# MicahZoltu/lodestar

Measured on AMD Instinct MI355X. Metric: verified signature sets/sec (mainnet attestation mix), higher is better.
Workload: dtype u32 (381-bit Montgomery; device products on 14x28-bit limbs); 1 GPU; c3: gossip attestation flood, 6 slot(s) per batch, 7 batches in flight per GPU; slots_per_batch=6, sets_per_gpu=116736, jobs_per_gpu=104448, pubkeys_per_gpu=1683456, parallelism=dp1 (sets sharded), exchange=False, inflight=7, world_size_seen=1, pubkeys=indices into the GPU-resident table, signing_roots_per_gpu=6918

## Files before the change

lodestar_amd/csrc/lb_curve.h:

```cpp
#pragma once
#include "lb_field.h"

template <class F>
struct jac {
  F x, y, z;
};
template <class F>
struct aff {
  F x, y;
};

typedef jac<fp> g1j;
typedef jac<fp2> g2j;
typedef aff<fp> g1a;
typedef aff<fp2> g2a;

template <class T, class S>
LB_HD aff<T> aff_as(const aff<S>& a) {
  return aff<T>{T{a.x}, T{a.y}};
}
template <class T, class S>
LB_HD jac<T> jac_as(const jac<S>& a) {
  return jac<T>{T{a.x}, T{a.y}, T{a.z}};
}
// ... 214 lines not shown
  }
  return acc;
}

template <class F>
LB_NI jac<F> jac_mul_u64_jac(jac<F> p, uint64_t k) {
  jac<F> acc = jac_infinity<F>();
  for (int i = 63; i >= 0; i--) {
    acc = jac_dbl_i(acc);
    if ((k >> i) & 1ull) acc = jac_add_i(acc, p);
  }
  return acc;
}

template <class F>
LB_NI jac<F> jac_mul_u256(aff<F> p, const uint32_t* k) {
  jac<F> acc = jac_infinity<F>();
  for (int i = 255; i >= 0; i--) {
    acc = jac_dbl_i(acc);
    if ((k[i >> 5] >> (i & 31)) & 1u) acc = jac_add_aff_i(acc, p);
  }
  return acc;
}

template <class F, bool kInl = false>
LB_HD jac<F> jac_mul_xabs_i(const jac<F>& p) {
  jac<F> acc = p;
  for (int i = 62; i >= 0; i--) {
    acc = jac_dbl_i(acc);
    if ((LB_X_ABS >> i) & 1ull) acc = jac_add_i<F, kInl>(acc, p);
  }
  return acc;
}
template <class F>
LB_NI jac<F> jac_mul_xabs(jac<F> p) {
  return jac_mul_xabs_i(p);
}

LB_HD g2j g2_psi(const g2j& p) {
  g2j r;
  r.x = fp2_mul(fp2_conj(p.x), fp2_load(LB_PSI_CX));
  r.y = fp2_mul(fp2_conj(p.y), fp2_load(LB_PSI_CY));
  r.z = fp2_conj(p.z);
  return r;
}
LB_HD g2j g2_psi2(const g2j& p) {
  g2j r;
  r.x = fp2_mul_fp(p.x, fp_load(LB_PSI2_CX));
  r.y = fp2_mul_fp(p.y, fp_load(LB_PSI2_CY));
  r.z = p.z;
  return r;
}

LB_HD bool g2_in_subgroup(const g2j& p) {
  if (jac_is_inf(p)) return true;
  g2j xp = jac_neg(jac_mul_xabs(p));
  return jac_eq(g2_psi(p), xp);
}

template <bool kInl>
LB_HD fp lean_mul(const fp& a, const fp& b) {
#if defined(__HIP_DEVICE_COMPILE__)
  if constexpr (kInl) {
    __builtin_amdgcn_sched_barrier(0);
    fp r = fp_mul28(a, b);
    __builtin_amdgcn_sched_barrier(0);
    return r;
  }
#endif
  return fp_mul(a, b);
}
template <bool kInl>
LB_HD fp lean_sqr(const fp& a) {
#if defined(__HIP_DEVICE_COMPILE__)
  if constexpr (kInl) {
    __builtin_amdgcn_sched_barrier(0);
    fp r = fp_sqr28(a);
    __builtin_amdgcn_sched_barrier(0);
    return r;
  }
#endif
  return fp_sqr(a);
}
template <bool kInl>
LB_HD fp2 lean2_mul(const fp2& a, const fp2& b) {
  fp t0 = lean_mul<kInl>(a.c0, b.c0);
  fp t1 = lean_mul<kInl>(a.c1, b.c1);
  fp t2 = lean_mul<kInl>(fp_add(a.c0, a.c1), fp_add(b.c0, b.c1));
  return fp2{fp_sub(t0, t1), fp_sub(fp_sub(t2, t0), t1)};
}
template <bool kInl>
LB_HD fp2 lean2_sqr(const fp2& a) {
  fp t0 = lean_mul<kInl>(fp_add(a.c0, a.c1), fp_sub(a.c0, a.c1));
  fp t1 = lean_mul<kInl>(a.c0, a.c1);
  return fp2{t0, fp_dbl(t1)};
}
template <bool kInl>
LB_HD void g2_dbl_lean(g2j& p) {
  p.z = fp2_dbl(lean2_mul<kInl>(p.y, p.z));
  fp2 B = lean2_sqr<kInl>(p.y);
  fp2 C = lean2_sqr<kInl>(B);
  fp2 A = lean2_sqr<kInl>(p.x);
  fp2 D = lean2_sqr<kInl>(fp2_add(p.x, B));
  D = fp2_dbl(fp2_sub(fp2_sub(D, A), C));
  fp2 E = fp2_mul3(A);
  p.x = fp2_sub(lean2_sqr<kInl>(E), fp2_dbl(D));
  p.y = fp2_sub(lean2_mul<kInl>(E, fp2_sub(D, p.x)), fp2_mul8(C));
}
template <bool kInl>
LB_HD void g2_add_aff_lean(g2j& p, const g2a& q) {
  fp2 Z1Z1 = lean2_sqr<kInl>(p.z);
  fp2 H = fp2_sub(lean2_mul<kInl>(q.x, Z1Z1), p.x);
  fp2 rr = lean2_mul<kInl>(lean2_mul<kInl>(q.y, p.z), Z1Z1);
  rr = fp2_dbl(fp2_sub(rr, p.y));
  if (fp2_is_zero(H)) {
    if (fp2_is_zero(rr)) {
      g2_dbl_lean<kInl>(p);
    } else {
      p = jac_infinity<fp2>();
    }
    return;
  }
  fp2 HH = lean2_sqr<kInl>(H);
  p.z = fp2_sub(fp2_sub(lean2_sqr<kInl>(fp2_add(p.z, H)), Z1Z1), HH);
  fp2 I = fp2_mul4(HH);
  fp2 J = lean2_mul<kInl>(H, I);
  fp2 V = lean2_mul<kInl>(p.x, I);
  fp2 YJ = fp2_dbl(lean2_mul<kInl>(p.y, J));
  p.x = fp2_sub(fp2_sub(lean2_sqr<kInl>(rr), J), fp2_dbl(V));
  p.y = fp2_sub(lean2_mul<kInl>(rr, fp2_sub(V, p.x)), YJ);
}

template <bool kInl>
LB_HD void g2_add_lean(g2j& p, const g2j& q) {
  if (jac_is_inf(q)) return;
  if (jac_is_inf(p)) {
    p = q;
    return;
  }
  const fp2 Z1Z1 = lean2_sqr<kInl>(p.z), Z2Z2 = lean2_sqr<kInl>(q.z);
  const fp2 ZZ = fp2_sub(fp2_sub(lean2_sqr<kInl>(fp2_add(p.z, q.z)), Z1Z1), Z2Z2);
  const fp2 U1 = lean2_mul<kInl>(p.x, Z2Z2);
  const fp2 S1 = lean2_mul<kInl>(lean2_mul<kInl>(p.y, q.z), Z2Z2);
  const fp2 H = fp2_sub(lean2_mul<kInl>(q.x, Z1Z1), U1);
  const fp2 rr = fp2_dbl(fp2_sub(lean2_mul<kInl>(lean2_mul<kInl>(q.y, p.z), Z1Z1), S1));
  if (fp2_is_zero(H)) {
    if (fp2_is_zero(rr)) {
      p = q;
      g2_dbl_lean<kInl>(p);
    } else {
      p = jac_infinity<fp2>();
    }
    return;
  }
  p.z = lean2_mul<kInl>(ZZ, H);
  const fp2 I = lean2_sqr<kInl>(fp2_dbl(H));
  const fp2 J = lean2_mul<kInl>(H, I);
  const fp2 V = lean2_mul<kInl>(U1, I);
  p.x = fp2_sub(fp2_sub(lean2_sqr<kInl>(rr), J), fp2_dbl(V));
  p.y = fp2_sub(lean2_mul<kInl>(rr, fp2_sub(V, p.x)), fp2_dbl(lean2_mul<kInl>(S1, J)));
}

LB_HD bool g2_aff_in_subgroup_i(const g2a& a) {
  g2j acc = jac_from_aff(a);
#pragma clang loop unroll(disable)
  for (int i = 62; i >= 0; i--) {
    acc = jac_dbl_i(acc);
    if ((LB_X_ABS >> i) & 1ull) acc = jac_add_aff_i<fp2, true>(acc, a);
  }
  if (jac_is_inf(acc)) return false;
  fp2 z2 = fp2_sqr(acc.z);
  fp2 px = fp2_mul(fp2_conj(a.x), fp2_load(LB_PSI_CX));
  if (!fp2_eq(fp2_mul(px, z2), acc.x)) return false;
  fp2 py = fp2_mul(fp2_conj(a.y), fp2_load(LB_PSI_CY));
  return fp2_eq(fp2_mul(fp2_mul(py, z2), acc.z), fp2_neg(acc.y));
}

LB_NI g2j g2_clear_cofactor(g2j p) {
  g2j t1 = jac_neg(jac_mul_xabs(p));
  g2j t2 = g2_psi(p);
  g2j t3 = g2_psi2(jac_dbl(p));
  t3 = jac_add(t3, jac_neg(t2));
  t2 = jac_add(t1, t2);
  t2 = jac_neg(jac_mul_xabs(t2));
  t3 = jac_add(t3, t2);
  t3 = jac_add(t3, jac_neg(t1));
  return jac_add(t3, jac_neg(p));
}

LB_HD bool g1_aff_on_curve(const g1a& a) {
// ... 6 lines not shown
```

lodestar_amd/csrc/lb_field.h:

```cpp
#pragma once
#include "lb_common.h"
#include "lb_consts.h"

struct fp {
  uint32_t v[12];
};
struct fp2 {
  fp c0, c1;
};
struct fp6 {
  fp2 c0, c1, c2;
};
struct fp12 {
  fp6 c0, c1;
};

LB_HD fp fp_load(const uint32_t* c) {
  fp r;
  LB_UNROLL for (int i = 0; i < 12; i++) r.v[i] = c[i];
  return r;
}
LB_HD fp2 fp2_load(const uint32_t* c) {
  fp2 r;
  r.c0 = fp_load(c);
// ... 681 lines not shown
    }
    lb_sub_in(u, v);
    bool zero = true;
    LB_UNROLL for (int j = 0; j < 12; j++) zero &= u[j] == 0;
    if (zero) return false;
  }
}

LB_HD bool fp_plain_gt_half(const fp& plain) {
  uint32_t br = 0;
  LB_UNROLL for (int j = 0; j < 12; j++) {
    uint64_t d = (uint64_t)LB_HALF_P[j] - plain.v[j] - br;
    br = (uint32_t)(d >> 63);
  }
  return br != 0;
}

LB_HD bool fp_plain_from_be48(fp& out, const uint8_t* b, uint8_t first_byte_mask) {
  LB_UNROLL for (int i = 0; i < 12; i++) {
    int o = 44 - 4 * i;
    uint32_t b0 = b[o];
    if (i == 11) b0 &= first_byte_mask;
    out.v[i] = (b0 << 24) | ((uint32_t)b[o + 1] << 16) | ((uint32_t)b[o + 2] << 8) | b[o + 3];
  }
  const uint32_t Pl[12] = {LB_P0, LB_P1, LB_P2, LB_P3, LB_P4, LB_P5, LB_P6, LB_P7, LB_P8, LB_P9, LB_P10, LB_P11};
  uint32_t br = 0;
  LB_UNROLL for (int j = 0; j < 12; j++) {
    uint64_t d = (uint64_t)out.v[j] - Pl[j] - br;
    br = (uint32_t)(d >> 63);
  }
  return br != 0;
}

LB_HD uint32_t lb_bswap32(uint32_t x) { return (x >> 24) | ((x >> 8) & 0xff00u) | ((x << 8) & 0xff0000u) | (x << 24); }
LB_HD bool fp_plain_from_be48_w(fp& out, const uint32_t* w, uint8_t first_byte_mask) {
  LB_UNROLL for (int i = 0; i < 12; i++) out.v[i] = lb_bswap32(w[11 - i]);
  out.v[11] &= ((uint32_t)first_byte_mask << 24) | 0x00ffffffu;
  const uint32_t Pl[12] = {LB_P0, LB_P1, LB_P2, LB_P3, LB_P4, LB_P5, LB_P6, LB_P7, LB_P8, LB_P9, LB_P10, LB_P11};
  uint32_t br = 0;
  LB_UNROLL for (int j = 0; j < 12; j++) {
    uint64_t d = (uint64_t)out.v[j] - Pl[j] - br;
    br = (uint32_t)(d >> 63);
  }
  return br != 0;
}

LB_HD void fp_plain_to_be48(uint8_t* b, const fp& plain) {
  LB_UNROLL for (int i = 0; i < 12; i++) {
    int o = 44 - 4 * i;
    uint32_t w = plain.v[i];
    b[o] = (uint8_t)(w >> 24);
    b[o + 1] = (uint8_t)(w >> 16);
    b[o + 2] = (uint8_t)(w >> 8);
    b[o + 3] = (uint8_t)w;
  }
}

LB_HD fp2 fp2_zero() { return fp2{fp_zero(), fp_zero()}; }
LB_HD fp2 fp2_one() { return fp2{fp_one(), fp_zero()}; }
LB_HD bool fp2_is_zero(const fp2& a) { return fp_is_zero(a.c0) && fp_is_zero(a.c1); }
LB_HD bool fp2_eq(const fp2& a, const fp2& b) { return fp_eq(a.c0, b.c0) && fp_eq(a.c1, b.c1); }
LB_HD fp2 fp2_select(bool c, const fp2& a, const fp2& b) { return fp2{fp_select(c, a.c0, b.c0), fp_select(c, a.c1, b.c1)}; }
LB_HD fp2 fp2_add(const fp2& a, const fp2& b) { return fp2{fp_add(a.c0, b.c0), fp_add(a.c1, b.c1)}; }
LB_HD fp2 fp2_sub(const fp2& a, const fp2& b) { return fp2{fp_sub(a.c0, b.c0), fp_sub(a.c1, b.c1)}; }
LB_HD fp2 fp2_dbl(const fp2& a) { return fp2{fp_dbl(a.c0), fp_dbl(a.c1)}; }
LB_HD fp2 fp2_neg(const fp2& a) { return fp2{fp_neg(a.c0), fp_neg(a.c1)}; }
LB_HD fp2 fp2_conj(const fp2& a) { return fp2{a.c0, fp_neg(a.c1)}; }
LB_HD fp2 fp2_mul_fp(const fp2& a, const fp& s) { return fp2{fp_mul(a.c0, s), fp_mul(a.c1, s)}; }
LB_HD fp2 fp2_mul3(const fp2& a) { return fp2{fp_mul3(a.c0), fp_mul3(a.c1)}; }
LB_HD fp2 fp2_mul4(const fp2& a) { return fp2{fp_mul4(a.c0), fp_mul4(a.c1)}; }
LB_HD fp2 fp2_mul8(const fp2& a) { return fp2{fp_mul8(a.c0), fp_mul8(a.c1)}; }

LB_HD fp2 fp2_mul(const fp2& a, const fp2& b) {
  fp t0 = fp_mul(a.c0, b.c0);
  fp t1 = fp_mul(a.c1, b.c1);
  fp t2 = fp_mul(fp_add(a.c0, a.c1), fp_add(b.c0, b.c1));
  return fp2{fp_sub(t0, t1), fp_sub(fp_sub(t2, t0), t1)};
}
LB_HD fp2 fp2_sqr(const fp2& a) {
  fp t0 = fp_mul(fp_add(a.c0, a.c1), fp_sub(a.c0, a.c1));
  fp t1 = fp_mul(a.c0, a.c1);
  return fp2{t0, fp_dbl(t1)};
}
LB_HD fp2 fp2_mul_xi(const fp2& a) { return fp2{fp_sub(a.c0, a.c1), fp_add(a.c0, a.c1)}; }

LB_NI fp2 fp2_inv(fp2 a) {
  fp n = fp_add(fp_sqr(a.c0), fp_sqr(a.c1));
  fp ni = fp_inv(n);
  return fp2{fp_mul(a.c0, ni), fp_neg(fp_mul(a.c1, ni))};
}

LB_HD bool fp2_is_square(const fp2& a) { return fp_is_square(fp_add(fp_sqr(a.c0), fp_sqr(a.c1))); }

template <bool kInl = false>
LB_HD bool fp2_sqrt_i(fp2& out, const fp2& a) {
  fp norm = fp_add(fp_sqr(a.c0), fp_sqr(a.c1));
  fp alpha;
  if constexpr (kInl) alpha = fp_pow_const_i<true>(norm, LB_EXP_SQRT, 378);
  else alpha = fp_sqrt_cand(norm);
  fp inv2 = fp_load(LB_INV2);
  fp d1 = fp_mul(fp_add(a.c0, alpha), inv2);
  fp d2 = fp_mul(fp_sub(a.c0, alpha), inv2);
  fp delta = fp_select(fp_is_zero(d1), d2, d1);
  fp z;
  if constexpr (kInl) z = fp_pow_const_i<true>(delta, LB_EXP_ISQRT, 378);
  else z = fp_isqrt_cand(delta);
  fp s = fp_mul(delta, z);
  bool delta_qr = fp_eq(fp_sqr(s), delta);
  fp t = fp_mul(z, inv2);
  if (!delta_qr) t = fp_neg(t);
  fp q = fp_mul(a.c1, t);
  out.c0 = fp_select(delta_qr, s, q);
  out.c1 = fp_select(delta_qr, q, s);
  return fp2_eq(fp2_sqr(out), a);
}
LB_NI bool fp2_sqrt(fp2& out, fp2 a) { return fp2_sqrt_i(out, a); }
template <class Pow>
LB_HD bool fp2_sqrt_p(fp2& out, const fp2& a, Pow pow) {
  const fp norm = fp_add(fp_sqr(a.c0), fp_sqr(a.c1));
  const fp alpha = pow(norm, LB_EXP_SQRT, 378);
  const fp inv2 = fp_load(LB_INV2);
  const fp d1 = fp_mul(fp_add(a.c0, alpha), inv2);
  const fp d2 = fp_mul(fp_sub(a.c0, alpha), inv2);
  const fp delta = fp_select(fp_is_zero(d1), d2, d1);
  const fp z = pow(delta, LB_EXP_ISQRT, 378);
  const fp s = fp_mul(delta, z);
  const bool delta_qr = fp_eq(fp_sqr(s), delta);
  fp t = fp_mul(z, inv2);
  if (!delta_qr) t = fp_neg(t);
  const fp q = fp_mul(a.c1, t);
  out.c0 = fp_select(delta_qr, s, q);
  out.c1 = fp_select(delta_qr, q, s);
  return fp2_eq(fp2_sqr(out), a);
}

LB_HD uint32_t fp2_sgn0(const fp2& a) {
  fp p0 = fp_from_mont(a.c0), p1 = fp_from_mont(a.c1);
  uint32_t sign0 = p0.v[0] & 1u;
  uint32_t zero0 = fp_is_zero(p0) ? 1u : 0u;
  uint32_t sign1 = p1.v[0] & 1u;
  return sign0 | (zero0 & sign1);
}

LB_HD bool fp2_lex_larger(const fp2& a) {
  fp p0 = fp_from_mont(a.c0), p1 = fp_from_mont(a.c1);
  return fp_is_zero(p1) ? fp_plain_gt_half(p0) : fp_plain_gt_half(p1);
}

LB_HD fp6 fp6_zero() { return fp6{fp2_zero(), fp2_zero(), fp2_zero()}; }
LB_HD fp6 fp6_one() { return fp6{fp2_one(), fp2_zero(), fp2_zero()}; }
LB_HD fp6 fp6_add(const fp6& a, const fp6& b) { return fp6{fp2_add(a.c0, b.c0), fp2_add(a.c1, b.c1), fp2_add(a.c2, b.c2)}; }
LB_HD fp6 fp6_sub(const fp6& a, const fp6& b) { return fp6{fp2_sub(a.c0, b.c0), fp2_sub(a.c1, b.c1), fp2_sub(a.c2, b.c2)}; }
LB_HD fp6 fp6_neg(const fp6& a) { return fp6{fp2_neg(a.c0), fp2_neg(a.c1), fp2_neg(a.c2)}; }
LB_HD fp6 fp6_mul_v(const fp6& a) { return fp6{fp2_mul_xi(a.c2), a.c0, a.c1}; }

LB_HD fp6 fp6_mul_inl(const fp6& a, const fp6& b) {
  fp2 t0 = fp2_mul(a.c0, b.c0);
  fp2 t1 = fp2_mul(a.c1, b.c1);
  fp2 t2 = fp2_mul(a.c2, b.c2);
  fp2 c0 = fp2_add(fp2_mul_xi(fp2_sub(fp2_sub(fp2_mul(fp2_add(a.c1, a.c2), fp2_add(b.c1, b.c2)), t1), t2)), t0);
  fp2 c1 = fp2_add(fp2_sub(fp2_sub(fp2_mul(fp2_add(a.c0, a.c1), fp2_add(b.c0, b.c1)), t0), t1), fp2_mul_xi(t2));
  fp2 c2 = fp2_add(fp2_sub(fp2_sub(fp2_mul(fp2_add(a.c0, a.c2), fp2_add(b.c0, b.c2)), t0), t2), t1);
  return fp6{c0, c1, c2};
}
LB_NI void fp6_mul_p(fp6* r, const fp6* pa, const fp6* pb) { *r = fp6_mul_inl(*pa, *pb); }
LB_HD fp6 fp6_mul(const fp6& a, const fp6& b) {
// ... 57 lines not shown
  fp12 r;
  fp12_sqr_p(&r, &a);
  return r;
}

LB_HD fp12 fp12_mul_line_inl(const fp12& a, const fp2& l0, const fp2& l2, const fp2& l3) {
  fp6 t0 = fp6_mul_01(a.c0, l0, l2);
  fp6 t1 = fp6_mul_1(a.c1, l3);
  fp6 c1 = fp6_sub(fp6_sub(fp6_mul_01(fp6_add(a.c0, a.c1), l0, fp2_add(l2, l3)), t0), t1);
  fp6 c0 = fp6_add(t0, fp6_mul_v(t1));
  return fp12{c0, c1};
}
LB_NI void fp12_mul_line_p(fp12* r, const fp12* pa, const fp2* pl0, const fp2* pl2, const fp2* pl3) {
  *r = fp12_mul_line_inl(*pa, *pl0, *pl2, *pl3);
}
LB_HD fp12 fp12_mul_line(const fp12& a, const fp2& l0, const fp2& l2, const fp2& l3) {
  fp12 r;
  fp12_mul_line_p(&r, &a, &l0, &l2, &l3);
  return r;
}

LB_NI fp12 fp12_inv(fp12 a) {
  fp6 t = fp6_sub(fp6_mul(a.c0, a.c0), fp6_mul_v(fp6_mul(a.c1, a.c1)));
  fp6 ti = fp6_inv(t);
  return fp12{fp6_mul(a.c0, ti), fp6_neg(fp6_mul(a.c1, ti))};
}

LB_NI fp12 fp12_frob(fp12 a) {
  fp12 r;
  r.c0.c0 = fp2_conj(a.c0.c0);
  r.c1.c0 = fp2_mul(fp2_conj(a.c1.c0), fp2_load(LB_FROB1_1));
  r.c0.c1 = fp2_mul(fp2_conj(a.c0.c1), fp2_load(LB_FROB1_2));
  r.c1.c1 = fp2_mul(fp2_conj(a.c1.c1), fp2_load(LB_FROB1_3));
  r.c0.c2 = fp2_mul(fp2_conj(a.c0.c2), fp2_load(LB_FROB1_4));
  r.c1.c2 = fp2_mul(fp2_conj(a.c1.c2), fp2_load(LB_FROB1_5));
  return r;
}
LB_NI fp12 fp12_frob2(fp12 a) {
  fp12 r;
  r.c0.c0 = a.c0.c0;
  r.c1.c0 = fp2_mul_fp(a.c1.c0, fp_load(LB_FROB2_1));
  r.c0.c1 = fp2_mul_fp(a.c0.c1, fp_load(LB_FROB2_2));
  r.c1.c1 = fp2_mul_fp(a.c1.c1, fp_load(LB_FROB2_3));
  r.c0.c2 = fp2_mul_fp(a.c0.c2, fp_load(LB_FROB2_4));
  r.c1.c2 = fp2_mul_fp(a.c1.c2, fp_load(LB_FROB2_5));
  return r;
}

LB_HD fp f_add(const fp& a, const fp& b) { return fp_add(a, b); }
LB_HD fp f_sub(const fp& a, const fp& b) { return fp_sub(a, b); }
LB_HD fp f_mul(const fp& a, const fp& b) { return fp_mul(a, b); }
LB_HD fp f_sqr(const fp& a) { return fp_sqr(a); }
LB_HD fp f_dbl(const fp& a) { return fp_dbl(a); }
LB_HD fp f_neg(const fp& a) { return fp_neg(a); }
LB_HD fp f_mul3(const fp& a) { return fp_mul3(a); }
LB_HD fp f_mul8(const fp& a) { return fp_mul8(a); }
LB_HD fp f_inv(const fp& a) { return fp_inv(a); }
LB_HD bool f_is_zero(const fp& a) { return fp_is_zero(a); }
LB_HD bool f_eq(const fp& a, const fp& b) { return fp_eq(a, b); }
LB_HD fp f_select(bool c, const fp& a, const fp& b) { return fp_select(c, a, b); }
LB_HD void f_set_zero(fp& a) { a = fp_zero(); }
LB_HD void f_set_one(fp& a) { a = fp_one(); }

struct fpi : fp {};
LB_HD fpi fpi_of(const fp& a) { return fpi{a}; }
LB_HD fpi f_add(const fpi& a, const fpi& b) { return fpi{fp_add(a, b)}; }
LB_HD fpi f_sub(const fpi& a, const fpi& b) { return fpi{fp_sub(a, b)}; }
LB_HD fpi f_mul(const fpi& a, const fpi& b) { return fpi{fp_mul_inl(a, b)}; }
LB_HD fpi f_sqr(const fpi& a) { return fpi{fp_sqr_inl(a)}; }
LB_HD fpi f_dbl(const fpi& a) { return fpi{fp_dbl(a)}; }
LB_HD fpi f_neg(const fpi& a) { return fpi{fp_neg(a)}; }
LB_HD fpi f_mul3(const fpi& a) { return fpi{fp_mul3(a)}; }
LB_HD fpi f_mul8(const fpi& a) { return fpi{fp_mul8(a)}; }
LB_HD bool f_is_zero(const fpi& a) { return fp_is_zero(a); }
LB_HD bool f_eq(const fpi& a, const fpi& b) { return fp_eq(a, b); }
LB_HD fpi f_select(bool c, const fpi& a, const fpi& b) { return fpi{fp_select(c, a, b)}; }
LB_HD void f_set_zero(fpi& a) { a = fpi{fp_zero()}; }
LB_HD void f_set_one(fpi& a) { a = fpi{fp_one()}; }

LB_HD fp2 f_add(const fp2& a, const fp2& b) { return fp2_add(a, b); }
struct fp2i : fp2 {};
LB_HD fp2i f_add(const fp2i& a, const fp2i& b) { return fp2i{fp2_add(a, b)}; }
LB_HD fp2i f_sub(const fp2i& a, const fp2i& b) { return fp2i{fp2_sub(a, b)}; }
LB_HD fp2i f_mul(const fp2i& a, const fp2i& b) {
  const fp t0 = fp_mul_inl(a.c0, b.c0);
  const fp t1 = fp_mul_inl(a.c1, b.c1);
  const fp t2 = fp_mul_inl(fp_add(a.c0, a.c1), fp_add(b.c0, b.c1));
  return fp2i{fp2{fp_sub(t0, t1), fp_sub(fp_sub(t2, t0), t1)}};
}
LB_HD fp2i f_sqr(const fp2i& a) {
  const fp t0 = fp_mul_inl(fp_add(a.c0, a.c1), fp_sub(a.c0, a.c1));
  const fp t1 = fp_mul_inl(a.c0, a.c1);
  return fp2i{fp2{t0, fp_dbl(t1)}};
}
LB_HD fp2i f_dbl(const fp2i& a) { return fp2i{fp2_dbl(a)}; }
LB_HD fp2i f_neg(const fp2i& a) { return fp2i{fp2_neg(a)}; }
LB_HD fp2i f_mul3(const fp2i& a) { return fp2i{fp2_mul3(a)}; }
LB_HD fp2i f_mul8(const fp2i& a) { return fp2i{fp2_mul8(a)}; }
LB_HD bool f_is_zero(const fp2i& a) { return fp2_is_zero(a); }
LB_HD bool f_eq(const fp2i& a, const fp2i& b) { return fp2_eq(a, b); }
LB_HD fp2i f_select(bool c, const fp2i& a, const fp2i& b) { return fp2i{fp2_select(c, a, b)}; }
LB_HD void f_set_zero(fp2i& a) { a = fp2i{fp2_zero()}; }
LB_HD void f_set_one(fp2i& a) { a = fp2i{fp2_one()}; }
LB_HD fp2 f_sub(const fp2& a, const fp2& b) { return fp2_sub(a, b); }
LB_HD fp2 f_mul(const fp2& a, const fp2& b) { return fp2_mul(a, b); }
LB_HD fp2 f_sqr(const fp2& a) { return fp2_sqr(a); }
LB_HD fp2 f_dbl(const fp2& a) { return fp2_dbl(a); }
LB_HD fp2 f_neg(const fp2& a) { return fp2_neg(a); }
LB_HD fp2 f_mul3(const fp2& a) { return fp2_mul3(a); }
LB_HD fp2 f_mul8(const fp2& a) { return fp2_mul8(a); }
LB_HD fp2 f_inv(const fp2& a) { return fp2_inv(a); }
LB_HD bool f_is_zero(const fp2& a) { return fp2_is_zero(a); }
LB_HD bool f_eq(const fp2& a, const fp2& b) { return fp2_eq(a, b); }
LB_HD fp2 f_select(bool c, const fp2& a, const fp2& b) { return fp2_select(c, a, b); }
LB_HD void f_set_zero(fp2& a) { a = fp2_zero(); }
LB_HD void f_set_one(fp2& a) { a = fp2_one(); }
```

lodestar_amd/csrc/lb_kernels.h:

```cpp
#pragma once
#include "lb_serial.h"
#include "lb_h2c.h"
#include "lb_pairing.h"

#define LB_TPB 64
#ifndef LB_MINW
#define LB_MINW 1
#endif
#ifndef LB_MINW_DEC
#define LB_MINW_DEC 2
#endif
#ifndef LB_MINW_SUB
#define LB_MINW_SUB LB_MINW_DEC
#endif
#ifndef LB_MINW_MSM
#define LB_MINW_MSM 1
#endif
#ifndef LB_MINW_GSUM
#define LB_MINW_GSUM 1
#endif
typedef fpi lb_g1f;
typedef fp2i lb_g2f;
typedef jac<lb_g2f> g2jm;
#ifndef LB_MINW_G1
// ... 78 lines not shown
  __shared__ uint32_t s_tot[NW][12];
  __shared__ uint32_t s_inv[12];
  const unsigned lane = threadIdx.x & 63u, wv = threadIdx.x >> 6;
  fp pre = z, suf = z;
  for (unsigned d = 1; d < 64; d <<= 1) {
    fp t = fp_shfl_up(pre, d);
    if (lane >= d) pre = fp_mul(pre, t);
  }
  for (unsigned d = 1; d < 64; d <<= 1) {
    fp t = fp_shfl_down(suf, d);
    if (lane + d < 64) suf = fp_mul(suf, t);
  }
  if (lane == 63) LB_UNROLL for (int j = 0; j < 12; j++) s_tot[wv][j] = pre.v[j];
  __syncthreads();
  if (wv == 0) {
    fp t = fp_load(s_tot[0]);
    for (int w = 1; w < NW; w++) t = fp_mul(t, fp_load(s_tot[w]));
    if constexpr (kInl) t = fp_inv_i(t);
    else t = fp_inv(t);
    if (lane == 0) LB_UNROLL for (int j = 0; j < 12; j++) s_inv[j] = t.v[j];
  }
  __syncthreads();
  fp winv = fp_load(s_inv);
  for (int w = 0; w < NW; w++)
    if (w != (int)wv) winv = fp_mul(winv, fp_load(s_tot[w]));
  fp pe = fp_shfl_up(pre, 1), se = fp_shfl_down(suf, 1);
  if (lane == 0) pe = fp_one();
  if (lane == 63) se = fp_one();
  return fp_mul(fp_mul(pe, se), winv);
}

#if LB_KG(0)
__global__ void __launch_bounds__(LB_TPB, LB_MINW_DEC) k_decompress_sigs(uint32_t n, const uint8_t* __restrict__ sigs,
                                                            const uint32_t* __restrict__ sig_sizes,
                                                            uint32_t* __restrict__ sig_aff,
                                                            uint4* __restrict__ sig_aos,
                                                            uint32_t* __restrict__ sig_inf,
                                                            int32_t* __restrict__ sig_status) {
  uint32_t i = lb_tid();
  if (i >= n) return;
  int st = LB_OK;
  g2a a;
  bool inf = false;
  if (sig_sizes != nullptr && sig_sizes[i] != 96) {
    st = LB_INVALID_SIZE;
    a.x = fp2_zero();
    a.y = fp2_zero();
  } else {
    uint32_t w[24];
    const uint4* s = reinterpret_cast<const uint4*>(sigs + (size_t)96 * i);
    LB_UNROLL for (int k = 0; k < 6; k++) {
      const uint4 v = s[k];
      w[4 * k] = v.x, w[4 * k + 1] = v.y, w[4 * k + 2] = v.z, w[4 * k + 3] = v.w;
    }
    st = g2_decompress96_w(w, a, inf);
  }
  soa_st(sig_aff, n, i, a);
  const uint32_t* w = reinterpret_cast<const uint32_t*>(&a);
  LB_UNROLL for (int k = 0; k < 12; k++) sig_aos[(size_t)12 * i + k] = make_uint4(w[4 * k], w[4 * k + 1], w[4 * k + 2], w[4 * k + 3]);
  sig_inf[i] = inf ? 1u : 0u;
  sig_status[i] = st;
}
#endif

#if LB_KG(1)
__global__ void __launch_bounds__(LB_TPB, LB_MINW_SUB) k_sig_subgroup(uint32_t n, const uint32_t* __restrict__ sig_aff,
                                                         const uint32_t* __restrict__ sig_inf,
                                                         int32_t* __restrict__ sig_status) {
  uint32_t i = lb_tid();
  if (i >= n) return;
  if (sig_status[i] != LB_OK || sig_inf[i]) return;
  auto load_f2 = [&](int o) {
    const uint32_t* base = sig_aff;
    asm volatile("" : "+s"(base));
    fp2 a;
    uint32_t* w = reinterpret_cast<uint32_t*>(&a);
    LB_UNROLL for (int k = 0; k < 24; k++) w[k] = __builtin_nontemporal_load(base + (size_t)(k + o) * n + i);
    return a;
  };
  g2j acc = jac_from_aff(g2a{load_f2(0), load_f2(24)});
  bool redo = false;
#pragma clang loop unroll(disable)
  for (int b = 62; b >= 0;) {
    g2_dbl_lean<true>(acc);
    if (redo) {
      redo = false;
      b--;
      continue;
    }
    if ((LB_X_ABS >> b) & 1ull) {
      if (jac_is_inf(acc)) {
        acc = jac_from_aff(g2a{load_f2(0), load_f2(24)});
        b--;
        continue;
      }
      const fp2 Z1Z1 = lean2_sqr<true>(acc.z);
      const fp2 H = fp2_sub(lean2_mul<true>(load_f2(0), Z1Z1), acc.x);
      const fp2 t = lean2_mul<true>(acc.z, Z1Z1);
      const fp2 rr = fp2_dbl(fp2_sub(lean2_mul<true>(load_f2(24), t), acc.y));
      if (fp2_is_zero(H)) {
        if (fp2_is_zero(rr)) {
          acc = jac_from_aff(g2a{load_f2(0), load_f2(24)});
          redo = true;
        } else {
          acc = jac_infinity<fp2>();
          b--;
        }
        continue;
      }
      acc.z = fp2_dbl(lean2_mul<true>(acc.z, H));
      const fp2 I = fp2_mul4(lean2_sqr<true>(H));
      const fp2 J = lean2_mul<true>(H, I);
      const fp2 V = lean2_mul<true>(acc.x, I);
      const fp2 YJ = fp2_dbl(lean2_mul<true>(acc.y, J));
      acc.x = fp2_sub(fp2_sub(lean2_sqr<true>(rr), J), fp2_dbl(V));
      acc.y = fp2_sub(lean2_mul<true>(rr, fp2_sub(V, acc.x)), YJ);
    }
    b--;
  }
  bool ok = !jac_is_inf(acc);
  if (ok) {
    const fp2 z2 = lean2_sqr<true>(acc.z);
    ok = fp2_eq(lean2_mul<true>(lean2_mul<true>(fp2_conj(load_f2(0)), fp2_load(LB_PSI_CX)), z2),
                acc.x);
    if (ok) {
      const fp2 py = lean2_mul<true>(fp2_conj(load_f2(24)), fp2_load(LB_PSI_CY));
      ok = fp2_eq(lean2_mul<true>(lean2_mul<true>(py, z2), acc.z), fp2_neg(acc.y));
    }
  }
  if (!ok) sig_status[i] = LB_POINT_NOT_IN_GROUP;
}
#endif

#if LB_KG(1)
__global__ void __launch_bounds__(64) k_sig_subgroup_g8(uint32_t n, const uint32_t* __restrict__ sig_aff,
                                                        const uint32_t* __restrict__ sig_inf,
                                                        int32_t* __restrict__ sig_status) {
  __shared__ uint32_t g8s[8 * 72];
  const uint32_t i = blockIdx.x * 8 + (threadIdx.x >> 3);
  if (i >= n) return;
  if (sig_status[i] != LB_OK || sig_inf[i]) return;
  lds_u32* G = (lds_u32*)g8s + (threadIdx.x >> 3) * 72;
  g8_stash(G, 0, jac_from_aff(soa_ld<g2a>(sig_aff, n, i)));
  const g2j acc = g8_mul_xabs_st(G, 0);
  bool ok = !jac_is_inf(acc);
  if (ok) ok = jac_eq(g8_psi(g8_unstash(G, 0)), jac_neg(acc));
  if (!ok && g8_q() == 0) sig_status[i] = LB_POINT_NOT_IN_GROUP;
}
#endif

typedef uint32_t lb_v8u __attribute__((ext_vector_type(8)));
static __device__ __attribute__((noinline)) lb_v8u sha256_compress_v(lb_v8u hv, lb_v16u bv) {
  uint32_t h[8], blk[16];
  LB_UNROLL for (int i = 0; i < 8; i++) h[i] = hv[i];
  LB_UNROLL for (int i = 0; i < 16; i++) blk[i] = bv[i];
  sha256_compress(h, blk);
  lb_v8u r;
  LB_UNROLL for (int i = 0; i < 8; i++) r[i] = h[i];
  return r;
}
__device__ __forceinline__ uint32_t dst_byte(int k) { return k < LB_DST_LEN + 1 ? (uint32_t)LB_DST[k] : 0u; }
__device__ __forceinline__ uint32_t dst_word(int k) {
  return (dst_byte(k) << 24) | (dst_byte(k + 1) << 16) | (dst_byte(k + 2) << 8) | dst_byte(k + 3);
}
__device__ __forceinline__ lb_v8u sha256_iv_v() {
  lb_v8u h;
  h[0] = 0x6a09e667; h[1] = 0xbb67ae85; h[2] = 0x3c6ef372; h[3] = 0xa54ff53a;
  h[4] = 0x510e527f; h[5] = 0x9b05688c; h[6] = 0x1f83d9ab; h[7] = 0x5be0cd19;
  return h;
}
__device__ __forceinline__ fp2 hash_to_field_u(const uint32_t M[8], int which) {
  const lb_v8u iv = sha256_iv_v();
  lb_v16u blk;
  LB_UNROLL for (int i = 0; i < 16; i++) blk[i] = 0u;
  lb_v8u b0 = sha256_compress_v(iv, blk);
  LB_UNROLL for (int i = 0; i < 8; i++) blk[i] = M[i];
  blk[8] = 0x01000000u | dst_byte(0);
  LB_UNROLL for (int i = 9; i < 16; i++) blk[i] = dst_word(4 * i - 35);
  b0 = sha256_compress_v(b0, blk);
  LB_UNROLL for (int i = 0; i < 4; i++) blk[i] = dst_word(29 + 4 * i);
  blk[3] = (dst_byte(41) << 24) | (dst_byte(42) << 16) | (dst_byte(43) << 8) | 0x80u;
  LB_UNROLL for (int i = 4; i < 15; i++) blk[i] = 0u;
  blk[15] = 143u * 8u;
  b0 = sha256_compress_v(b0, blk);
  uint32_t out[32];
  lb_v8u prev = b0 ^ b0;
  LB_UNROLL for (int i = 1; i <= 8; i++) {
    if ((i - 1) / 4 > which) break;
    lb_v16u bb;
    LB_UNROLL for (int k = 0; k < 8; k++) bb[k] = b0[k] ^ prev[k];
    bb[8] = ((uint32_t)i << 24) | (dst_byte(0) << 16) | (dst_byte(1) << 8) | dst_byte(2);
    LB_UNROLL for (int k = 9; k < 16; k++) bb[k] = dst_word(4 * k - 33);
    lb_v8u bi = sha256_compress_v(iv, bb);
    LB_UNROLL for (int k = 0; k < 3; k++) bb[k] = dst_word(31 + 4 * k);
    bb[3] = (dst_byte(43) << 24) | 0x00800000u;
    LB_UNROLL for (int k = 4; k < 15; k++) bb[k] = 0u;
    bb[15] = 77u * 8u;
    bi = sha256_compress_v(bi, bb);
    prev = bi;
    if ((i - 1) / 4 == which) LB_UNROLL for (int k = 0; k < 8; k++) out[8 * ((i - 1) & 3) + k] = bi[k];
  }
  return fp2{fp_from_be64_words(out), fp_from_be64_words(out + 16)};
}
__device__ __forceinline__ fp2 fp2_inv_i(const fp2& a) {
  const fp ni = fp_inv_i(fp_add(fp_sqr(a.c0), fp_sqr(a.c1)));
  return fp2{fp_mul(a.c0, ni), fp_neg(fp_mul(a.c1, ni))};
}
__device__ __forceinline__ bool fp_is_square_bin_i(const fp& a) {
  if (fp_is_zero(a)) return true;
  uint32_t u[12], v[12];
// ... 2379 lines not shown
```

Before: 11.91 million sets/s.

## Fuse Fp2 Montgomery multiply and square with lazy 28-bit column reduction

Adds fused Fp2 multiply and square routines on 14x28-bit limbs. Each one accumulates the Karatsuba sub-products column by column in signed 64-bit accumulators and interleaves a single Montgomery reduction per component, instead of running three separate Fp multiplies plus adds and subs. The new routines are used in the G2 subgroup-check kernel and for every fp2i multiply and square, so the G2 MSM and other inlined-field paths change too. This removes duplicate reductions and intermediate repacking, at the cost of larger unrolled code, higher register pressure and reliance on column-bound analysis (a host-side overflow checker is included).

```diff
diff --git a/lodestar_amd/csrc/lb_curve.h b/lodestar_amd/csrc/lb_curve.h
--- a/lodestar_amd/csrc/lb_curve.h
+++ b/lodestar_amd/csrc/lb_curve.h
@@ -320,30 +320,32 @@
 #endif
   return fp_sqr(a);
 }
-template <bool kInl>
+template <bool kInl, bool kLazy = false>
 LB_HD fp2 lean2_mul(const fp2& a, const fp2& b) {
+  if constexpr (kInl && kLazy) return fp2_mul28_lazy(a, b);
   fp t0 = lean_mul<kInl>(a.c0, b.c0);
   fp t1 = lean_mul<kInl>(a.c1, b.c1);
   fp t2 = lean_mul<kInl>(fp_add(a.c0, a.c1), fp_add(b.c0, b.c1));
   return fp2{fp_sub(t0, t1), fp_sub(fp_sub(t2, t0), t1)};
 }
-template <bool kInl>
+template <bool kInl, bool kLazy = false>
 LB_HD fp2 lean2_sqr(const fp2& a) {
+  if constexpr (kInl && kLazy) return fp2_sqr28_lazy(a);
   fp t0 = lean_mul<kInl>(fp_add(a.c0, a.c1), fp_sub(a.c0, a.c1));
   fp t1 = lean_mul<kInl>(a.c0, a.c1);
   return fp2{t0, fp_dbl(t1)};
 }
-template <bool kInl>
+template <bool kInl, bool kLazy = false>
 LB_HD void g2_dbl_lean(g2j& p) {
-  p.z = fp2_dbl(lean2_mul<kInl>(p.y, p.z));
-  fp2 B = lean2_sqr<kInl>(p.y);
-  fp2 C = lean2_sqr<kInl>(B);
-  fp2 A = lean2_sqr<kInl>(p.x);
-  fp2 D = lean2_sqr<kInl>(fp2_add(p.x, B));
+  p.z = fp2_dbl(lean2_mul<kInl, kLazy>(p.y, p.z));
+  fp2 B = lean2_sqr<kInl, kLazy>(p.y);
+  fp2 C = lean2_sqr<kInl, kLazy>(B);
+  fp2 A = lean2_sqr<kInl, kLazy>(p.x);
+  fp2 D = lean2_sqr<kInl, kLazy>(fp2_add(p.x, B));
   D = fp2_dbl(fp2_sub(fp2_sub(D, A), C));
   fp2 E = fp2_mul3(A);
-  p.x = fp2_sub(lean2_sqr<kInl>(E), fp2_dbl(D));
-  p.y = fp2_sub(lean2_mul<kInl>(E, fp2_sub(D, p.x)), fp2_mul8(C));
+  p.x = fp2_sub(lean2_sqr<kInl, kLazy>(E), fp2_dbl(D));
+  p.y = fp2_sub(lean2_mul<kInl, kLazy>(E, fp2_sub(D, p.x)), fp2_mul8(C));
 }
 template <bool kInl>
 LB_HD void g2_add_aff_lean(g2j& p, const g2a& q) {
diff --git a/lodestar_amd/csrc/lb_field.h b/lodestar_amd/csrc/lb_field.h
--- a/lodestar_amd/csrc/lb_field.h
+++ b/lodestar_amd/csrc/lb_field.h
@@ -787,6 +787,137 @@
   fp t1 = fp_mul(a.c0, a.c1);
   return fp2{t0, fp_dbl(t1)};
 }
+#if defined(LB_FP2_LAZY_CHECK) && !defined(__HIPCC__)
+#include <stdlib.h>
+struct lb_col {
+  __int128 v;
+  lb_col() : v(0) {}
+  lb_col(__int128 x) : v(x) {
+    if (x > (__int128)INT64_MAX || x < (__int128)INT64_MIN) abort();
+  }
+  lb_col operator+(const lb_col& o) const { return lb_col(v + o.v); }
+  lb_col operator-(const lb_col& o) const { return lb_col(v - o.v); }
+  lb_col& operator+=(const lb_col& o) { return *this = *this + o; }
+  lb_col operator>>(int s) const { return lb_col(v >> s); }
+  lb_col operator<<(int s) const { return lb_col(v * ((__int128)1 << s)); }
+  explicit operator uint32_t() const { return (uint32_t)v; }
+};
+LB_HD lb_col lb_colp(uint32_t a, uint32_t b) { return lb_col((__int128)((uint64_t)a * b)); }
+#else
+typedef int64_t lb_col;
+LB_HD lb_col lb_colp(uint32_t a, uint32_t b) { return (lb_col)((uint64_t)a * b); }
+#endif
+LB_HD void lb_lazy_fence() {
+#if defined(__HIP_DEVICE_COMPILE__)
+  __builtin_amdgcn_sched_barrier(0);
+#endif
+}
+LB_HD void lb_lazy_pin(lb_col& c) {
+#if defined(__HIP_DEVICE_COMPILE__)
+  asm("" : "+v"(c));
+#endif
+}
+template <int sh>
+LB_HD void lb_unpack28(uint32_t* A, const fp& a) {
+  A[0] = (a.v[0] << sh) & 0x0fffffffu;
+  LB_UNROLL for (int k = 1; k < 14; k++) A[k] = lb_bits28(a.v, 28 * k - sh);
+}
+LB_HD fp lb_repack28(const uint32_t* r, int nsub) {
+  uint32_t o[12];
+  LB_UNROLL for (int w = 0; w < 12; w++) {
+    const int l = (32 * w) / 28, s = 32 * w - 28 * l;
+    o[w] = (r[l] >> s) | (r[l + 1] << (28 - s));
+  }
+  fp c = fp_reduce_once(o, 0u);
+  if (nsub > 1) c = fp_reduce_once(c.v, 0u);
+  return c;
+}
+LB_HD void lb_lazy_col(lb_col& c, uint32_t* m, uint32_t* r, int k) {
+  const uint32_t P28[14] = {LB_P28_0, LB_P28_1, LB_P28_2, LB_P28_3, LB_P28_4,  LB_P28_5,  LB_P28_6,
+                            LB_P28_7, LB_P28_8, LB_P28_9, LB_P28_10, LB_P28_11, LB_P28_12, LB_P28_13};
+  LB_UNROLL for (int i = (k > 13 ? k - 13 : 0); i < k && i < 14; i++) {
+    c += lb_colp(m[i], P28[k - i]);
+    lb_lazy_pin(c);
+  }
+  if (k < 14) {
+    m[k] = ((uint32_t)c * LB_PINV28) & 0x0fffffffu;
+    c += lb_colp(m[k], P28[0]);
+  } else {
+    r[k - 14] = (uint32_t)c & 0x0fffffffu;
+  }
+  c = c >> 28;
+}
+LB_HD fp2 fp2_mul28_lazy(const fp2& a, const fp2& b) {
+  const uint32_t P28[14] = {LB_P28_0, LB_P28_1, LB_P28_2, LB_P28_3, LB_P28_4,  LB_P28_5,  LB_P28_6,
+                            LB_P28_7, LB_P28_8, LB_P28_9, LB_P28_10, LB_P28_11, LB_P28_12, LB_P28_13};
+  LB_COUNT_MUL(), LB_COUNT_MUL(), LB_COUNT_MUL();
+  lb_lazy_fence();
+  uint32_t A0[14], A1[14], B0[14], B1[14], As[14], Bs[14];
+  lb_unpack28<0>(A0, a.c0);
+  lb_unpack28<0>(A1, a.c1);
+  lb_unpack28<8>(B0, b.c0);
+  lb_unpack28<8>(B1, b.c1);
+  LB_UNROLL for (int k = 0; k < 14; k++) As[k] = A0[k] + A1[k], Bs[k] = B0[k] + B1[k];
+  uint32_t m0[14], m1[14], r0[14], r1[14];
+  lb_col c0 = 0, c1 = 0;
+  LB_UNROLL for (int k = 0; k < 28; k++) {
+    lb_col t0 = 0, t1 = 0;
+    LB_UNROLL for (int i = (k > 13 ? k - 13 : 0); i <= k && i < 14; i++) {
+      t0 += lb_colp(A0[i], B0[k - i]);
+      t1 += lb_colp(A1[i], B1[k - i]);
+      c1 += lb_colp(As[i], Bs[k - i]);
+    }
+    c0 += t0 - t1;
+    if (k >= 14) c0 += lb_col(P28[k - 14]);
+    c1 += lb_col(0) - (t0 + t1);
+    lb_lazy_col(c0, m0, r0, k);
+    lb_lazy_col(c1, m1, r1, k);
+  }
+  fp2 c;
+  c.c0 = lb_repack28(r0, 2);
+  c.c1 = lb_repack28(r1, 1);
+  lb_lazy_fence();
+  return c;
+}
+LB_HD fp2 fp2_sqr28_lazy(const fp2& a) {
+  const uint32_t P28[14] = {LB_P28_0, LB_P28_1, LB_P28_2, LB_P28_3, LB_P28_4,  LB_P28_5,  LB_P28_6,
+                            LB_P28_7, LB_P28_8, LB_P28_9, LB_P28_10, LB_P28_11, LB_P28_12, LB_P28_13};
+  LB_COUNT_MUL(), LB_COUNT_MUL();
+  lb_lazy_fence();
+  uint32_t A0[14], A1[14], As[14];
+  uint32_t D0[14], D1[14], Ds[14];
+  lb_unpack28<4>(A0, a.c0);
+  lb_unpack28<4>(A1, a.c1);
+  LB_UNROLL for (int k = 0; k < 14; k++) {
+    As[k] = A0[k] + A1[k];
+    D0[k] = A0[k] << 1, D1[k] = A1[k] << 1, Ds[k] = As[k] << 1;
+  }
+  uint32_t m0[14], m1[14], r0[14], r1[14];
+  lb_col c0 = 0, c1 = 0;
+  LB_UNROLL for (int k = 0; k < 28; k++) {
+    lb_col t0 = 0, t1 = 0, u = 0;
+    LB_UNROLL for (int i = (k > 13 ? k - 13 : 0); 2 * i < k; i++) {
+      t0 += lb_colp(D0[i], A0[k - i]);
+      t1 += lb_colp(D1[i], A1[k - i]);
+      u += lb_colp(Ds[i], As[k - i]);
+    }
+    if (k % 2 == 0 && k < 27) {
+      t0 += lb_colp(A0[k / 2], A0[k / 2]);
+      t1 += lb_colp(A1[k / 2], A1[k / 2]);
+      u += lb_colp(As[k / 2], As[k / 2]);
+    }
+    c0 += t0 - t1;
+    if (k >= 14) c0 += lb_col(P28[k - 14]);
+    c1 += u - (t0 + t1);
+    lb_lazy_col(c0, m0, r0, k);
+    lb_lazy_col(c1, m1, r1, k);
+  }
+  fp2 c;
+  c.c0 = lb_repack28(r0, 2);
+  c.c1 = lb_repack28(r1, 1);
+  lb_lazy_fence();
+  return c;
+}
 LB_HD fp2 fp2_mul_xi(const fp2& a) { return fp2{fp_sub(a.c0, a.c1), fp_add(a.c0, a.c1)}; }
 
 LB_NI fp2 fp2_inv(fp2 a) {
@@ -1010,17 +1141,8 @@
 struct fp2i : fp2 {};
 LB_HD fp2i f_add(const fp2i& a, const fp2i& b) { return fp2i{fp2_add(a, b)}; }
 LB_HD fp2i f_sub(const fp2i& a, const fp2i& b) { return fp2i{fp2_sub(a, b)}; }
-LB_HD fp2i f_mul(const fp2i& a, const fp2i& b) {
-  const fp t0 = fp_mul_inl(a.c0, b.c0);
-  const fp t1 = fp_mul_inl(a.c1, b.c1);
-  const fp t2 = fp_mul_inl(fp_add(a.c0, a.c1), fp_add(b.c0, b.c1));
-  return fp2i{fp2{fp_sub(t0, t1), fp_sub(fp_sub(t2, t0), t1)}};
-}
-LB_HD fp2i f_sqr(const fp2i& a) {
-  const fp t0 = fp_mul_inl(fp_add(a.c0, a.c1), fp_sub(a.c0, a.c1));
-  const fp t1 = fp_mul_inl(a.c0, a.c1);
-  return fp2i{fp2{t0, fp_dbl(t1)}};
-}
+LB_HD fp2i f_mul(const fp2i& a, const fp2i& b) { return fp2i{fp2_mul28_lazy(a, b)}; }
+LB_HD fp2i f_sqr(const fp2i& a) { return fp2i{fp2_sqr28_lazy(a)}; }
 LB_HD fp2i f_dbl(const fp2i& a) { return fp2i{fp2_dbl(a)}; }
 LB_HD fp2i f_neg(const fp2i& a) { return fp2i{fp2_neg(a)}; }
 LB_HD fp2i f_mul3(const fp2i& a) { return fp2i{fp2_mul3(a)}; }
diff --git a/lodestar_amd/csrc/lb_kernels.h b/lodestar_amd/csrc/lb_kernels.h
--- a/lodestar_amd/csrc/lb_kernels.h
+++ b/lodestar_amd/csrc/lb_kernels.h
@@ -184,7 +184,7 @@
   bool redo = false;
 #pragma clang loop unroll(disable)
   for (int b = 62; b >= 0;) {
-    g2_dbl_lean<true>(acc);
+    g2_dbl_lean<true, true>(acc);
     if (redo) {
       redo = false;
       b--;
@@ -196,10 +196,10 @@
         b--;
         continue;
       }
-      const fp2 Z1Z1 = lean2_sqr<true>(acc.z);
-      const fp2 H = fp2_sub(lean2_mul<true>(load_f2(0), Z1Z1), acc.x);
-      const fp2 t = lean2_mul<true>(acc.z, Z1Z1);
-      const fp2 rr = fp2_dbl(fp2_sub(lean2_mul<true>(load_f2(24), t), acc.y));
+      const fp2 Z1Z1 = lean2_sqr<true, true>(acc.z);
+      const fp2 H = fp2_sub(lean2_mul<true, true>(load_f2(0), Z1Z1), acc.x);
+      const fp2 t = lean2_mul<true, true>(acc.z, Z1Z1);
+      const fp2 rr = fp2_dbl(fp2_sub(lean2_mul<true, true>(load_f2(24), t), acc.y));
       if (fp2_is_zero(H)) {
         if (fp2_is_zero(rr)) {
           acc = jac_from_aff(g2a{load_f2(0), load_f2(24)});
@@ -210,24 +210,24 @@
         }
         continue;
       }
-      acc.z = fp2_dbl(lean2_mul<true>(acc.z, H));
-      const fp2 I = fp2_mul4(lean2_sqr<true>(H));
-      const fp2 J = lean2_mul<true>(H, I);
-      const fp2 V = lean2_mul<true>(acc.x, I);
-      const fp2 YJ = fp2_dbl(lean2_mul<true>(acc.y, J));
-      acc.x = fp2_sub(fp2_sub(lean2_sqr<true>(rr), J), fp2_dbl(V));
-      acc.y = fp2_sub(lean2_mul<true>(rr, fp2_sub(V, acc.x)), YJ);
+      acc.z = fp2_dbl(lean2_mul<true, true>(acc.z, H));
+      const fp2 I = fp2_mul4(lean2_sqr<true, true>(H));
+      const fp2 J = lean2_mul<true, true>(H, I);
+      const fp2 V = lean2_mul<true, true>(acc.x, I);
+      const fp2 YJ = fp2_dbl(lean2_mul<true, true>(acc.y, J));
+      acc.x = fp2_sub(fp2_sub(lean2_sqr<true, true>(rr), J), fp2_dbl(V));
+      acc.y = fp2_sub(lean2_mul<true, true>(rr, fp2_sub(V, acc.x)), YJ);
     }
     b--;
   }
   bool ok = !jac_is_inf(acc);
   if (ok) {
-    const fp2 z2 = lean2_sqr<true>(acc.z);
-    ok = fp2_eq(lean2_mul<true>(lean2_mul<true>(fp2_conj(load_f2(0)), fp2_load(LB_PSI_CX)), z2),
+    const fp2 z2 = lean2_sqr<true, true>(acc.z);
+    ok = fp2_eq(lean2_mul<true, true>(lean2_mul<true, true>(fp2_conj(load_f2(0)), fp2_load(LB_PSI_CX)), z2),
                 acc.x);
     if (ok) {
-      const fp2 py = lean2_mul<true>(fp2_conj(load_f2(24)), fp2_load(LB_PSI_CY));
-      ok = fp2_eq(lean2_mul<true>(lean2_mul<true>(py, z2), acc.z), fp2_neg(acc.y));
+      const fp2 py = lean2_mul<true, true>(fp2_conj(load_f2(24)), fp2_load(LB_PSI_CY));
+      ok = fp2_eq(lean2_mul<true, true>(lean2_mul<true, true>(py, z2), acc.z), fp2_neg(acc.y));
     }
   }
   if (!ok) sig_status[i] = LB_POINT_NOT_IN_GROUP;
```

Measured after the change: 12.17 million sets/s, median of 6. No clear change (+2.1%).
